# 1pathplanningzzj/pointnet_refine

Measured on AMD Instinct MI355X. Metric: lane segments/sec (fwd+bwd) at B=4096,N=1024; HBM GB/s vs roofline, higher is better.
Workload: dtype f32 (large GEMMs: 2xfp16-split MFMA, 3 products, fp32 accumulate); 1 GPU; LineRefineNet training step (fwd + deep-supervision L1 + bwd + Adam), B=4096/GPU, N=1024, M=32, C=4; global_batch=4096, points=1024, parallelism=dp1, decoder_chunk=4096

## Files before the change

### pointnet_refine_amd/csrc/prh_attn16.hpp

```cpp
#pragma once
#include "prh_attn.hpp"
#include "prh_gemm_h2.hpp"

namespace prh {

constexpr int A16_ROWB = 80;
constexpr int A16_IMG = 32 * A16_ROWB;

template <int PREC> struct A16 {
  static constexpr int NPL = PREC == 0 ? 2 : 1;
  using frag = typename std::conditional<PREC == 0, f16x8, bf16x8>::type;
};

template <int PREC>
__device__ __forceinline__ float a16_scale(const float (&x)[16]) {
  if constexpr (PREC != 0) return 1.f;
  float m = 0.f;
#pragma unroll
  for (int t = 0; t < 16; ++t) m = fmaxf(m, fabsf(x[t]));
#pragma unroll
  for (int o = 32; o > 0; o >>= 1) m = fmaxf(m, __shfl_xor(m, o));
  return pow2_scale(m);
}
__device__ __forceinline__ float a16_scale_acc(const f32x16& x) {
  float m = 0.f;
#pragma unroll
  for (int t = 0; t < 16; ++t) m = fmaxf(m, fabsf(x[t]));
#pragma unroll
  for (int o = 32; o > 0; o >>= 1) m = fmaxf(m, __shfl_xor(m, o));
  return pow2_scale(m);
}
template <int PREC, int NP>
__device__ __forceinline__ void a16_split(const float* x_, typename A16<PREC>::frag (&o)[NP], float S = 1.f) {
  if constexpr (PREC == 0 && NP == 1) {
    typedef float v2f __attribute__((ext_vector_type(2)));
    uint4 h;
    unsigned* hp = reinterpret_cast<unsigned*>(&h);
#pragma unroll
    for (int j = 0; j < 4; ++j) {
      v2f v = {x_[2 * j] * S, x_[2 * j + 1] * S};
      f16x2 hb = __builtin_convertvector(v, f16x2);
      hp[j] = __builtin_bit_cast(unsigned, hb);
    }
    o[0] = __builtin_bit_cast(f16x8, h);
  } else if constexpr (PREC == 0) {
    float x[8];
#pragma unroll
    for (int j = 0; j < 8; ++j) x[j] = x_[j] * S;
    uint4 h, l;
    split2h(x[0], x[1], h.x, l.x); split2h(x[2], x[3], h.y, l.y);
    split2h(x[4], x[5], h.z, l.z); split2h(x[6], x[7], h.w, l.w);
    o[0] = __builtin_bit_cast(f16x8, h);
    o[1] = __builtin_bit_cast(f16x8, l);
  } else {
    const uint4 h = make_uint4(pack_bf16x2(x_[0], x_[1]), pack_bf16x2(x_[2], x_[3]), pack_bf16x2(x_[4], x_[5]),
                               pack_bf16x2(x_[6], x_[7]));
    o[0] = __builtin_bit_cast(bf16x8, h);
  }
}
template <int PREC, int NA, int NB>
__device__ __forceinline__ f32x16 a16_mma(const typename A16<PREC>::frag (&a)[NA],
                                          const typename A16<PREC>::frag (&b)[NB], f32x16 c) {
  if constexpr (PREC == 0) {
    if constexpr (NA > 1) c = __builtin_amdgcn_mfma_f32_32x32x16_f16(a[NA - 1], b[0], c, 0, 0, 0);
    if constexpr (NB > 1) c = __builtin_amdgcn_mfma_f32_32x32x16_f16(a[0], b[NB - 1], c, 0, 0, 0);
    c = __builtin_amdgcn_mfma_f32_32x32x16_f16(a[0], b[0], c, 0, 0, 0);
  } else {
    c = __builtin_amdgcn_mfma_f32_32x32x16_bf16(a[0], b[0], c, 0, 0, 0);
  }
  return c;
}
__device__ __forceinline__ void a16_load_rows(const float* base, long ld, long row0, int rows_valid, int col0,
                                              int lane, float (&x)[16]) {
  const int r = lane & 31, h2 = lane >> 5;
  const bool ok = r < rows_valid;
  const float* p = base + (size_t)(row0 + (ok ? r : 0)) * ld + col0 + h2 * 8;
#pragma unroll
  for (int s = 0; s < 2; ++s)
#pragma unroll
    for (int j = 0; j < 2; ++j) {
      const float4 t = ok ? ldg4(p + s * 16 + 4 * j) : zero4();
      x[s * 8 + 4 * j] = t.x; x[s * 8 + 4 * j + 1] = t.y; x[s * 8 + 4 * j + 2] = t.z; x[s * 8 + 4 * j + 3] = t.w;
    }
}
template <bool KV16>
__device__ __forceinline__ void a16_load_kv(const float* base, long ld, long row0, int rows_valid, int col0,
                                            int lane, float (&x)[16]) {
  if constexpr (!KV16) {
    a16_load_rows(base, ld, row0, rows_valid, col0, lane, x);
  } else {
    const int r = lane & 31, h2 = lane >> 5;
    const bool ok = r < rows_valid;
    const unsigned short* p = reinterpret_cast<const unsigned short*>(base) + (size_t)(row0 + (ok ? r : 0)) * ld + col0 + h2 * 8;
#pragma unroll
    for (int s = 0; s < 2; ++s) {
      const uint4 u = ok ? *reinterpret_cast<const uint4*>(p + s * 16) : make_uint4(0u, 0u, 0u, 0u);
      x[s * 8 + 0] = bf16_lo(u.x); x[s * 8 + 1] = bf16_hi(u.x); x[s * 8 + 2] = bf16_lo(u.y); x[s * 8 + 3] = bf16_hi(u.y);
      x[s * 8 + 4] = bf16_lo(u.z); x[s * 8 + 5] = bf16_hi(u.z); x[s * 8 + 6] = bf16_lo(u.w); x[s * 8 + 7] = bf16_hi(u.w);
    }
  }
}
template <int PREC, int NP>
__device__ __forceinline__ void a16_store_rows(char* img, int lane, const typename A16<PREC>::frag (&f0)[NP],
                                               const typename A16<PREC>::frag (&f1)[NP]) {
  const int r = lane & 31, h2 = lane >> 5;
#pragma unroll
  for (int pl = 0; pl < NP; ++pl) {
    char* q = img + pl * A16_IMG + r * A16_ROWB + h2 * 16;
    *reinterpret_cast<uint4*>(q) = __builtin_bit_cast(uint4, f0[pl]);
    *reinterpret_cast<uint4*>(q + 32) = __builtin_bit_cast(uint4, f1[pl]);
  }
  asm volatile("" ::: "memory");
}
template <int PREC, int NP>
__device__ __forceinline__ void a16_tr(const char* img, int s, int lane, typename A16<PREC>::frag (&o)[NP]) {
  const int g = lane >> 4, j = lane & 15;
  const char* a = img + (16 * s + 4 * (g >> 1) + (j >> 2)) * A16_ROWB + (16 * (g & 1) + 4 * (j & 3)) * 2;
#pragma unroll
  for (int pl = 0; pl < NP; ++pl) {
    const fp16x4 lo = __builtin_amdgcn_ds_read_tr16_b64_v4f16((__attribute__((address_space(3))) fp16x4*)(a + pl * A16_IMG));
    const fp16x4 hi = __builtin_amdgcn_ds_read_tr16_b64_v4f16(
        (__attribute__((address_space(3))) fp16x4*)(a + pl * A16_IMG + 8 * A16_ROWB));
    struct Pair { fp16x4 a, b; } pr = {lo, hi};
    o[pl] = __builtin_bit_cast(typename A16<PREC>::frag, pr);
  }
}
template <int PREC, int NP>
__device__ __forceinline__ void a16_acc_frag(const f32x16& x, int s, typename A16<PREC>::frag (&o)[NP],
                                             float S = 1.f) {
  float t[8];
#pragma unroll
  for (int j = 0; j < 8; ++j) t[j] = x[8 * s + j];
  a16_split<PREC>(t, o, S);
}
__device__ __forceinline__ f32x16 a16_zero() {
  f32x16 z;
#pragma unroll
  for (int r = 0; r < 16; ++r) z[r] = 0.f;
  return z;
}

template <int PREC> constexpr int a16_fwd_wave_lds() {
  return A16<PREC>::NPL * A16_IMG > 18 * 64 * 4 ? A16<PREC>::NPL * A16_IMG : 18 * 64 * 4;
}
template <int PREC, bool KV16 = false>
__global__ __launch_bounds__(512) void attn16_fwd_kernel(const AttnParams p) {
  using frag = typename A16<PREC>::frag;
  constexpr int NPL = A16<PREC>::NPL;
  constexpr int NKV = KV16 ? 1 : NPL;
  constexpr int WL = a16_fwd_wave_lds<PREC>();
  extern __shared__ __attribute__((aligned(16))) char smem[];
  const int lane = threadIdx.x & 63, wave = threadIdx.x >> 6;
  const int h2 = lane >> 5, l31 = lane & 31;
  const int wpb = blockDim.x >> 6;
  const int hpb = p.H / wpb;
  const bool split = p.ksplit > 0;
  const int b = split ? blockIdx.x / p.H : blockIdx.x / hpb;
  const int h = split ? blockIdx.x % p.H : (blockIdx.x % hpb) * wpb + wave;
  const int kbeg = split ? wave * p.ksplit : 0;
  int kend = split ? kbeg + p.ksplit : p.N;
  kend = kend > p.N ? p.N : kend;
  const unsigned seed_eff = effective_seed(p.seed, p.seed_src);
  char* vimg = smem + wave * WL;
  const int col0 = h * 32;
  const unsigned bh = (unsigned)(b * p.H + h);

  for (int qt = 0; qt < p.M; qt += 32) {
    float x[16];
    a16_load_rows(p.q, p.ldq, (long)b * p.M + qt, p.M - qt, col0, lane, x);
#pragma unroll
    for (int t = 0; t < 16; ++t) x[t] *= p.scale;
    const float sq = a16_scale<PREC>(x);
    frag qf[2][NPL];
    a16_split<PREC>(x, qf[0], sq);
    a16_split<PREC>(x + 8, qf[1], sq);

    f32x16 oacc;
#pragma unroll
    for (int r = 0; r < 16; ++r) oacc[r] = 0.f;
    float m_run = -INFINITY, l_run = 0.f;

    float kn[16], vn[16];
    if (kbeg < kend) {
      a16_load_kv<KV16>(p.k, p.ldk, (long)b * p.N + kbeg, p.N - kbeg, col0, lane, kn);
      a16_load_kv<KV16>(p.v, p.ldv, (long)b * p.N + kbeg, p.N - kbeg, col0, lane, vn);
    }
    for (int k0 = kbeg; k0 < kend; k0 += 32) {
      frag kf[2][NKV], vf[2][NKV];
      const float sk = a16_scale<PREC>(kn), sv = a16_scale<PREC>(vn);
      a16_split<PREC>(kn, kf[0], sk); a16_split<PREC>(kn + 8, kf[1], sk);
      a16_split<PREC>(vn, vf[0], sv); a16_split<PREC>(vn + 8, vf[1], sv);
      if (k0 + 32 < kend) {
        a16_load_kv<KV16>(p.k, p.ldk, (long)b * p.N + k0 + 32, p.N - k0 - 32, col0, lane, kn);
        a16_load_kv<KV16>(p.v, p.ldv, (long)b * p.N + k0 + 32, p.N - k0 - 32, col0, lane, vn);
      }
      a16_store_rows<PREC>(vimg, lane, vf[0], vf[1]);
      f32x16 s = a16_zero();
      s = a16_mma<PREC>(kf[0], qf[0], s);
      s = a16_mma<PREC>(kf[1], qf[1], s);
      const float us = 1.f / (sk * sq);
      float mx = -INFINITY;
#pragma unroll
      for (int r = 0; r < 16; ++r) {
        s[r] = (k0 + crow(r, h2) >= p.N) ? -INFINITY : s[r] * us;
        mx = fmaxf(mx, s[r]);
      }
      mx = fmaxf(mx, __shfl_xor(mx, 32));
      const float m_new = fmaxf(m_run, mx);
      const float alpha = __expf(m_run - m_new);
      float psum = 0.f;
#pragma unroll
      for (int r = 0; r < 16; ++r) {
        const float e = __expf(s[r] - m_new);
        psum += e;
        float pd = e;
        if (p.drop_thresh != 0u)
          pd = attn_keep(seed_eff, bh, (unsigned)(qt + l31), (unsigned)(k0 + crow(r, h2)), p.drop_thresh)
                   ? e * p.keep_scale : 0.f;
        s[r] = pd;
        oacc[r] *= alpha;
      }
      psum += __shfl_xor(psum, 32);
      l_run = l_run * alpha + psum;
      m_run = m_new;
      f32x16 ot = a16_zero();
#pragma unroll
      for (int st = 0; st < 2; ++st) {
        frag pf[NPL], va[NKV];
        a16_acc_frag<PREC>(s, st, pf);
        a16_tr<PREC>(vimg, st, lane, va);
        ot = a16_mma<PREC>(va, pf, ot);
      }
      const float uv = 1.f / sv;
#pragma unroll
      for (int r = 0; r < 16; ++r) oacc[r] = fmaf(ot[r], uv, oacc[r]);
    }
    const int q = qt + l31;
    if (split) {
      asm volatile("" ::: "memory");
      float* part = reinterpret_cast<float*>(vimg);
#pragma unroll
      for (int r = 0; r < 16; ++r) part[r * 64 + lane] = oacc[r];
      part[16 * 64 + lane] = m_run;
      part[17 * 64 + lane] = l_run;
      __syncthreads();
      for (int g = wave; g < 4; g += wpb) {
        float mt = -INFINITY;
        for (int sw = 0; sw < wpb; ++sw) mt = fmaxf(mt, reinterpret_cast<const float*>(smem + sw * WL)[16 * 64 + lane]);
        float lt = 0.f;
        float4 ov = zero4();
        for (int sw = 0; sw < wpb; ++sw) {
          const float* ps = reinterpret_cast<const float*>(smem + sw * WL);
          const float ms = ps[16 * 64 + lane];
          const float w = ms == -INFINITY ? 0.f : __expf(ms - mt);
          lt = fmaf(ps[17 * 64 + lane], w, lt);
          ov.x = fmaf(ps[(4 * g) * 64 + lane], w, ov.x); ov.y = fmaf(ps[(4 * g + 1) * 64 + lane], w, ov.y);
          ov.z = fmaf(ps[(4 * g + 2) * 64 + lane], w, ov.z); ov.w = fmaf(ps[(4 * g + 3) * 64 + lane], w, ov.w);
        }
        const float inv = 1.f / lt;
        if (q < p.M) {
          float* op = p.o + (size_t)((long)b * p.M + q) * p.ldo + col0;
          *reinterpret_cast<float4*>(op + 8 * g + 4 * h2) = make_float4(ov.x * inv, ov.y * inv, ov.z * inv, ov.w * inv);
          if (g == 0 && h2 == 0) p.lse[((size_t)b * p.H + h) * p.M + q] = mt + __logf(lt);
        }
      }
      __syncthreads();
      continue;
    }
    const float inv = 1.f / l_run;
    if (q < p.M) {
      float* op = p.o + (size_t)((long)b * p.M + q) * p.ldo + col0;
#pragma unroll
      for (int g = 0; g < 4; ++g)
        *reinterpret_cast<float4*>(op + 8 * g + 4 * h2) =
            make_float4(oacc[4 * g] * inv, oacc[4 * g + 1] * inv, oacc[4 * g + 2] * inv, oacc[4 * g + 3] * inv);
      if (h2 == 0) p.lse[((size_t)b * p.H + h) * p.M + q] = m_run + __logf(l_run);
    }
  }
}

template <int PREC, bool KV16 = false, bool KSPLIT = false>
__global__ __launch_bounds__(KSPLIT ? 512 : 256, KSPLIT ? 1 : 2) void attn16_bwd_kernel(const AttnParams p) {
  using frag = typename A16<PREC>::frag;
  constexpr int NPL = A16<PREC>::NPL;
  constexpr int NKV = KV16 ? 1 : NPL;
  constexpr bool SCR_IN_DS = AT_TILE * 4 <= NPL * A16_IMG;
  constexpr int WAVE_LDS = 4 * NPL * A16_IMG + (SCR_IN_DS ? 0 : AT_TILE * 4);
  extern __shared__ __attribute__((aligned(16))) char dsm16[];
  const int lane = threadIdx.x & 63, wave = threadIdx.x >> 6;
  const int h2 = lane >> 5, l31 = lane & 31;
  const int wpb = blockDim.x >> 6;
  const int hpb = p.H / wpb;
  constexpr bool split = KSPLIT;
  const int b = split ? blockIdx.x / p.H : blockIdx.x / hpb;
  const int h = split ? blockIdx.x % p.H : (blockIdx.x % hpb) * wpb + wave;
  const int kbeg = split ? wave * p.ksplit : 0;
  int kend = split ? kbeg + p.ksplit : p.N;
  kend = kend > p.N ? p.N : kend;
  const unsigned seed_eff = effective_seed(p.seed, p.seed_src);
  char* qimg = dsm16 + wave * WAVE_LDS;
  char* doimg = qimg + NPL * A16_IMG;
  char* kimg = doimg + NPL * A16_IMG;
  char* dsimg = kimg + NPL * A16_IMG;
  float* scr = reinterpret_cast<float*>(SCR_IN_DS ? dsimg : dsimg + NPL * A16_IMG);
  const int col0 = h * 32;
  const unsigned bh = (unsigned)(b * p.H + h);
  float mx_dv = 0.f, mx_dk = 0.f;

  for (int qt = 0; qt < p.M; qt += 32) {
    float xq[16], xdo[16], xo[16];
    a16_load_rows(p.q, p.ldq, (long)b * p.M + qt, p.M - qt, col0, lane, xq);
    a16_load_rows(p.dout, p.lddo, (long)b * p.M + qt, p.M - qt, col0, lane, xdo);
    a16_load_rows(p.o, p.ldo, (long)b * p.M + qt, p.M - qt, col0, lane, xo);
#pragma unroll
    for (int t = 0; t < 16; ++t) xq[t] *= p.scale;
    const float sq = a16_scale<PREC>(xq), sdo = a16_scale<PREC>(xdo);
    frag qf[2][NPL], dof[2][NPL];
    a16_split<PREC>(xq, qf[0], sq); a16_split<PREC>(xq + 8, qf[1], sq);
    a16_split<PREC>(xdo, dof[0], sdo); a16_split<PREC>(xdo + 8, dof[1], sdo);
    a16_store_rows<PREC>(qimg, lane, qf[0], qf[1]);
    a16_store_rows<PREC>(doimg, lane, dof[0], dof[1]);
    float dl = 0.f;
#pragma unroll
    for (int t = 0; t < 16; ++t) dl = fmaf(xdo[t], xo[t], dl);
    dl += __shfl_xor(dl, 32);
    const int qcol = qt + l31;
    const float lse_col = qcol < p.M ? p.lse[((size_t)b * p.H + h) * p.M + qcol] : 0.f;
    const float dl_col = dl;
    if (h2 == 0) *reinterpret_cast<float2*>(qimg + l31 * A16_ROWB + 64) = make_float2(lse_col, dl_col);
    asm volatile("" ::: "memory");
    f32x16 dqacc;
#pragma unroll
    for (int r = 0; r < 16; ++r) dqacc[r] = 0.f;

    float kn[16], vn[16];
    if (kbeg < kend) {
      a16_load_kv<KV16>(p.k, p.ldk, (long)b * p.N + kbeg, p.N - kbeg, col0, lane, kn);
      a16_load_kv<KV16>(p.v, p.ldv, (long)b * p.N + kbeg, p.N - kbeg, col0, lane, vn);
    }
    for (int k0 = kbeg; k0 < kend; k0 += 32) {
      frag kf[2][NKV], vf[2][NKV];
      const float sk = a16_scale<PREC>(kn), sv = a16_scale<PREC>(vn);
      a16_split<PREC>(kn, kf[0], sk); a16_split<PREC>(kn + 8, kf[1], sk);
      a16_split<PREC>(vn, vf[0], sv); a16_split<PREC>(vn + 8, vf[1], sv);
      if (k0 + 32 < kend) {
        a16_load_kv<KV16>(p.k, p.ldk, (long)b * p.N + k0 + 32, p.N - k0 - 32, col0, lane, kn);
        a16_load_kv<KV16>(p.v, p.ldv, (long)b * p.N + k0 + 32, p.N - k0 - 32, col0, lane, vn);
      }
      a16_store_rows<PREC>(kimg, lane, kf[0], kf[1]);
      const bool key_ok = (k0 + l31) < p.N;
      const float us = 1.f / (sq * sk), udp = 1.f / (sdo * sv);

      f32x16 s = a16_zero(), dp = a16_zero();
#pragma unroll
      for (int st = 0; st < 2; ++st) {
        s = a16_mma<PREC>(qf[st], kf[st], s);
        dp = a16_mma<PREC>(dof[st], vf[st], dp);
      }
#pragma unroll
      for (int r = 0; r < 16; ++r) {
        const int q = qt + crow(r, h2);
        const float2 qs = *reinterpret_cast<const float2*>(qimg + crow(r, h2) * A16_ROWB + 64);
        float pr = (key_ok && q < p.M) ? __expf(s[r] * us - qs.x) : 0.f;
        float keepf = 1.f;
        if (p.drop_thresh != 0u)
          keepf = attn_keep(seed_eff, bh, (unsigned)q, (unsigned)(k0 + l31), p.drop_thresh) ? p.keep_scale : 0.f;
        const float ds = pr * (dp[r] * udp * keepf - qs.y);
        s[r] = pr * keepf;
        dp[r] = ds;
      }
      f32x16 dvt = a16_zero(), dkt = a16_zero();
      const float sds = PREC == 0 ? a16_scale_acc(dp) : 1.f;
#pragma unroll
      for (int st = 0; st < 2; ++st) {
        frag pf[NPL], dsf[NPL], at[NPL];
        a16_acc_frag<PREC>(s, st, pf);
        a16_tr<PREC>(doimg, st, lane, at);
        dvt = a16_mma<PREC>(at, pf, dvt);
        a16_acc_frag<PREC>(dp, st, dsf, sds);
        a16_tr<PREC>(qimg, st, lane, at);
        dkt = a16_mma<PREC>(at, dsf, dkt);
#pragma unroll
        for (int pl = 0; pl < NPL; ++pl) {
          const uint4 u = __builtin_bit_cast(uint4, dsf[pl]);
          char* q = dsimg + pl * A16_IMG + l31 * A16_ROWB + (16 * st + 4 * h2) * 2;
          *reinterpret_cast<uint2*>(q) = make_uint2(u.x, u.y);
          *reinterpret_cast<uint2*>(q + 16) = make_uint2(u.z, u.w);
        }
      }
      asm volatile("" ::: "memory");
      {
        const float uv = 1.f / sdo, uk = 1.f / (sq * sds);
#pragma unroll
        for (int r = 0; r < 16; ++r) { dvt[r] *= uv; dkt[r] *= uk; }
      }
      {
        f32x16 dqt = a16_zero();
#pragma unroll
        for (int st = 0; st < 2; ++st) {
          frag bt[NPL], at[NKV];
          a16_tr<PREC>(dsimg, st, lane, bt);
          a16_tr<PREC>(kimg, st, lane, at);
          dqt = a16_mma<PREC>(at, bt, dqt);
        }
        const float uq = 1.f / (sk * sds);
#pragma unroll
        for (int r = 0; r < 16; ++r) dqacc[r] = fmaf(dqt[r], uq, dqacc[r]);
      }
      asm volatile("" ::: "memory");
#pragma unroll
      for (int pass = 0; pass < 2; ++pass) {
        const f32x16& acc = pass == 0 ? dvt : dkt;
#pragma unroll
        for (int r = 0; r < 16; ++r) scr[l31 * AT_LD + crow(r, h2)] = acc[r];
        float* dst = pass == 0 ? p.dv : p.dk;
        const long ldd = pass == 0 ? p.lddv : p.lddk;
#pragma unroll
        for (int it = 0; it < 4; ++it) {
          const int key = (lane >> 3) + 8 * it;
          float4 vv = *reinterpret_cast<const float4*>(scr + key * AT_LD + (lane & 7) * 4);
          if (k0 + key < p.N) {
            const size_t eo = (size_t)((long)b * p.N + k0 + key) * ldd + col0 + (lane & 7) * 4;
            if constexpr (KV16) {
              uint2* gp = reinterpret_cast<uint2*>(reinterpret_cast<unsigned short*>(dst) + eo);
              if (qt > 0) {
                const uint2 old = *gp;
                vv.x += bf16_lo(old.x); vv.y += bf16_hi(old.x); vv.z += bf16_lo(old.y); vv.w += bf16_hi(old.y);
              }
              *gp = make_uint2(pack_bf16x2(vv.x, vv.y), pack_bf16x2(vv.z, vv.w));
            } else {
              float* gp = dst + eo;
              if (qt > 0) {
                const float4 old = ldg4(gp);
                vv.x += old.x; vv.y += old.y; vv.z += old.z; vv.w += old.w;
              }
              *reinterpret_cast<float4*>(gp) = vv;
            }
            const float m4 = fmaxf(fmaxf(fabsf(vv.x), fabsf(vv.y)), fmaxf(fabsf(vv.z), fabsf(vv.w)));
            if (pass == 0) mx_dv = fmaxf(mx_dv, m4); else mx_dk = fmaxf(mx_dk, m4);
          }
        }
      }
    }
    if (split) {
      asm volatile("" ::: "memory");
#pragma unroll
      for (int r = 0; r < 16; ++r) scr[r * 64 + lane] = dqacc[r];
      __syncthreads();
      for (int g = wave; g < 4 && qcol < p.M; g += wpb) {
        float4 dv4 = zero4();
        for (int sw = 0; sw < wpb; ++sw) {
          const float* ps = reinterpret_cast<const float*>(dsm16 + sw * WAVE_LDS + (scr - reinterpret_cast<float*>(qimg)) * 4);
          dv4.x += ps[(4 * g) * 64 + lane]; dv4.y += ps[(4 * g + 1) * 64 + lane];
          dv4.z += ps[(4 * g + 2) * 64 + lane]; dv4.w += ps[(4 * g + 3) * 64 + lane];
        }
        float* dqp = p.dq + (size_t)((long)b * p.M + qcol) * p.lddq + col0;
        *reinterpret_cast<float4*>(dqp + 8 * g + 4 * h2) =
            make_float4(dv4.x * p.scale, dv4.y * p.scale, dv4.z * p.scale, dv4.w * p.scale);
      }
      __syncthreads();
    } else if (qcol < p.M) {
      float* dqp = p.dq + (size_t)((long)b * p.M + qcol) * p.lddq + col0;
#pragma unroll
      for (int g = 0; g < 4; ++g)
        *reinterpret_cast<float4*>(dqp + 8 * g + 4 * h2) =
            make_float4(dqacc[4 * g] * p.scale, dqacc[4 * g + 1] * p.scale, dqacc[4 * g + 2] * p.scale,
                        dqacc[4 * g + 3] * p.scale);
    }
  }
  if (p.kv_amax_part != nullptr) {
#pragma unroll
    for (int o = 32; o > 0; o >>= 1) {
      mx_dv = fmaxf(mx_dv, __shfl_xor(mx_dv, o));
      mx_dk = fmaxf(mx_dk, __shfl_xor(mx_dk, o));
    }
    if (split) {
      float* red = reinterpret_cast<float*>(dsm16);
      if (lane == 0) { red[wave * 2] = mx_dv; red[wave * 2 + 1] = mx_dk; }
      __syncthreads();
      if (threadIdx.x == 0) {
        for (int sw = 1; sw < wpb; ++sw) { mx_dv = fmaxf(mx_dv, red[sw * 2]); mx_dk = fmaxf(mx_dk, red[sw * 2 + 1]); }
        p.kv_amax_part[(size_t)blockIdx.x * 2] = mx_dv;
        p.kv_amax_part[(size_t)blockIdx.x * 2 + 1] = mx_dk;
      }
    } else if (lane == 0) {
      p.kv_amax_part[(size_t)(blockIdx.x * wpb + wave) * 2] = mx_dv;
      p.kv_amax_part[(size_t)(blockIdx.x * wpb + wave) * 2 + 1] = mx_dk;
    }
  }
}

}
```

### pointnet_refine_amd/csrc/prh_lib.hip

```cpp
#include "../../include/pointnet_refine_hip.h"

#include <hip/hip_runtime.h>
#include <stdarg.h>
#include <stdio.h>
#include <string.h>

#include <mutex>
#include <vector>

#include <stdlib.h>

#include "prh_gemm.hpp"
#include "prh_attn.hpp"
#include "prh_attn16.hpp"
#include "prh_gemm_s3.hpp"
#include "prh_gemm_h2.hpp"
#include "prh_b16.hpp"
#include "prh_small.hpp"
#include "prh_attnfold.hpp"
#include "prh_fused.hpp"
#include "prh_context.hpp"
#include "prh_metrics.hpp"
#include "prh_drive.hpp"
#include "prh_match.hpp"
// ... 3459 lines not shown
                     double cell, const long long* cell_offsets, const int* rows, long long n_rows, double r2,
                     double reach, double z_lo, double bin, int n_bins, int min_points, int peak_num, int peak_den,
                     double* height, int* count, int* hits, int* bin_index, int device, void* stream) {
  TRY_RC(ground_check_grid("ground_query", points, is_double, slice_offsets, n_slices, n_points, grid_origin, grid_shape,
                           cell_base, n_cells, cell));
  if (n_queries < 0 || n_queries >= 4ll * 0x7fffffff || n_rows < 0 || n_rows > n_points)
    return fail(PRH_ERR_ARG, "ground_query: bad argument");
  if (!(r2 > 0.0) || !(r2 <= 16.0) || !(reach > 0.0) || !(reach * reach >= r2) || !(reach <= 8.0))
    return fail(PRH_ERR_ARG, "ground_query: 0 < radius <= 4 and radius <= reach <= 8");
  if (n_bins < 1 || n_bins > GROUND_MAX_BINS || !(bin > 0.0) || !(z_lo >= -256.0) || !(z_lo + n_bins * bin <= 256.0))
    return fail(PRH_ERR_ARG, "ground_query: 1 <= n_bins <= %d, bin > 0 and the histogram inside [-256, 256]",
                GROUND_MAX_BINS);
  if (min_points < 1 || peak_num < 1 || peak_num > peak_den || peak_den > 65536)
    return fail(PRH_ERR_ARG, "ground_query: min_points >= 1 and 1 <= peak_num <= peak_den <= 65536");
  if (n_queries == 0) return PRH_OK;
  if (!queries || !query_offsets || n_slices == 0 || !height || !count || !hits || !bin_index ||
      (n_cells > 0 && !cell_offsets) || (n_rows > 0 && !rows))
    return fail(PRH_ERR_ARG, "ground_query: null pointer");
  HIP_TRY(hipSetDevice(device));
  hipStream_t st = (hipStream_t)stream;
  GroundParams prm{r2, reach, cell, z_lo, bin, n_bins, min_points, peak_num, peak_den};
  const unsigned nblk = (unsigned)((n_queries + GROUND_WAVES - 1) / GROUND_WAVES);
  if (is_double)
    hipLaunchKernelGGL(ground_query_kernel<double>, dim3(nblk), dim3(GROUND_THREADS), 0, st, (const double*)points,
                       slice_offsets, n_slices, queries, query_offsets, n_queries, grid_origin, grid_shape, cell_base,
                       cell_offsets, rows, n_rows, n_cells, prm, height, count, hits, bin_index);
  else
    hipLaunchKernelGGL(ground_query_kernel<float>, dim3(nblk), dim3(GROUND_THREADS), 0, st, (const float*)points,
                       slice_offsets, n_slices, queries, query_offsets, n_queries, grid_origin, grid_shape, cell_base,
                       cell_offsets, rows, n_rows, n_cells, prm, height, count, hits, bin_index);
  LAUNCH_CHECK();
  return PRH_OK;
}

static bool attn_ksplit(int B, int H, int N, int& keys_per_wave) {
  keys_per_wave = 0;
  if ((long)B * H > 1024 || N < 128) return false;
  int nw = cdiv(N, 32) < 8 ? cdiv(N, 32) : 8;
  keys_per_wave = cdiv(cdiv(N, 32), nw) * 32;
  return true;
}
static int attn_prepare(AttnParams& a, float dropout_p) {
  a.seed_src = g_seed_src;
  if (dropout_p < 0.f || dropout_p >= 1.f) return fail(PRH_ERR_ARG, "attention: dropout_p must be in [0,1)");
  a.keep_scale = 1.f / (1.f - dropout_p);
  a.drop_thresh = dropout_p > 0.f ? (unsigned)((double)dropout_p * 4294967296.0) : 0u;
  if (!a.q || !a.k || !a.v || !a.o || !a.lse || a.B <= 0 || a.M <= 0 || a.N <= 0)
    return fail(PRH_ERR_ARG, "attention: bad argument");
  if (a.H <= 0 || a.H % 4) return fail(PRH_ERR_ARG, "attention: heads (%d) must be a multiple of 4", a.H);
  if ((a.ldq | a.ldk | a.ldv | a.ldo) & 3) return fail(PRH_ERR_ARG, "attention: leading dimensions must be multiples of 4");
  return PRH_OK;
}

static int attn_forward(AttnParams& a, bool kv16, int prec, float dropout_p, int device, hipStream_t st) {
  TRY(attn_prepare(a, dropout_p));
  HIP_TRY(hipSetDevice(device));
  const int B = a.B, M = a.M, N = a.N, H = a.H;
  ProfScope ps(prec < 0 ? "attn_fwd" : "attn16_fwd<split>",
               4.0 * B * H * (double)M * N * 32, 4.0 * (2.0 * B * N * H * 32 + 2.0 * B * M * H * 32), st);
  int wpb = (long)B * (H / 4) < 512 ? 1 : 4;
  if (kv16 && prec < 0) return fail(PRH_ERR_ARG, "attention: bf16 K/V need the 16-bit attention cores");
  unsigned grid = (unsigned)(B * (H / wpb));
  if (prec >= 0 && attn_ksplit(B, H, N, a.ksplit)) { wpb = cdiv(N, a.ksplit); grid = (unsigned)(B * H); }
  const size_t ldsf = (size_t)wpb * a16_fwd_wave_lds<0>();
  if (prec >= 0 && kv16)
    hipLaunchKernelGGL((attn16_fwd_kernel<0, true>), dim3(grid), dim3(64 * wpb), ldsf, st, a);
  else if (prec >= 0)
    hipLaunchKernelGGL(attn16_fwd_kernel<0>, dim3(grid), dim3(64 * wpb), ldsf, st, a);
  else
    hipLaunchKernelGGL(attn_fwd_kernel, dim3(grid), dim3(64 * wpb), 0, st, a);
  LAUNCH_CHECK();
  return PRH_OK;
}

static int attn_backward(AttnParams& a, bool kv16, int prec, float dropout_p, int device, hipStream_t st) {
  TRY(attn_prepare(a, dropout_p));
  if (!a.dout || !a.dq || !a.dk || !a.dv) return fail(PRH_ERR_ARG, "attention_backward: null gradient pointer");
  if ((a.lddo | a.lddq | a.lddk | a.lddv) & 3) return fail(PRH_ERR_ARG, "attention_backward: leading dimensions must be multiples of 4");
  HIP_TRY(hipSetDevice(device));
  const int B = a.B, M = a.M, N = a.N, H = a.H;
  int wpb = (long)B * (H / 4) < 512 ? 1 : 4;
  if (prec >= 0) {
    unsigned grid = (unsigned)(B * (H / wpb));
    if (attn_ksplit(B, H, N, a.ksplit)) { wpb = cdiv(N, a.ksplit); grid = (unsigned)(B * H); }
    const size_t lds16 = (size_t)wpb * 4 * 2 * A16_IMG;
    static const int attr16 = allow_big_lds(attn16_bwd_kernel<0>, attn16_bwd_kernel<0, true>);
    if (attr16 != PRH_OK) return attr16;
    const double kvb = kv16 ? 2.0 : 4.0;
    ProfScope ps("attn16_bwd<split>", 14.0 * B * H * (double)M * N * 32,
                 kvb * 4.0 * B * N * H * 32 + 4.0 * 4.0 * B * M * H * 32, st);
    if (a.ksplit > 0) {
      static const int attr16s = allow_big_lds(attn16_bwd_kernel<0, false, true>, attn16_bwd_kernel<0, true, true>);
      if (attr16s != PRH_OK) return attr16s;
      if (kv16)
        hipLaunchKernelGGL((attn16_bwd_kernel<0, true, true>), dim3(grid), dim3(64 * wpb), lds16, st, a);
      else
        hipLaunchKernelGGL((attn16_bwd_kernel<0, false, true>), dim3(grid), dim3(64 * wpb), lds16, st, a);
    } else if (kv16)
      hipLaunchKernelGGL((attn16_bwd_kernel<0, true>), dim3(grid), dim3(64 * wpb), lds16, st, a);
    else
      hipLaunchKernelGGL(attn16_bwd_kernel<0>, dim3(grid), dim3(64 * wpb), lds16, st, a);
    LAUNCH_CHECK();
    return PRH_OK;
  }
  const size_t lds = (size_t)wpb * 4 * AT_TILE * sizeof(float);
  static const int attr_rc = allow_big_lds(attn_bwd_kernel);
  if (attr_rc != PRH_OK) return attr_rc;
  ProfScope ps("attn_bwd", 14.0 * B * H * (double)M * N * 32, 4.0 * (4.0 * B * N * H * 32 + 4.0 * B * M * H * 32), st);
  hipLaunchKernelGGL(attn_bwd_kernel, dim3((unsigned)(B * (H / wpb))), dim3(64 * wpb), lds, st, a);
  LAUNCH_CHECK();
  return PRH_OK;
}

int prh_attn_forward(const float* q, long ldq, const float* k, long ldk, const float* v, long ldv,
                     float* o, long ldo, float* lse, int B, int M, int N, int H, float scale,
                     float dropout_p, unsigned seed, int device, void* stream) {
  AttnParams a; memset(&a, 0, sizeof(a));
  a.q = q; a.ldq = ldq; a.k = k; a.ldk = ldk; a.v = v; a.ldv = ldv; a.o = o; a.ldo = ldo; a.lse = lse;
  a.B = B; a.M = M; a.N = N; a.H = H; a.scale = scale; a.seed = seed;
  return attn_forward(a, false, cores_of(gemm_mode()).attn_prec(), dropout_p, device, (hipStream_t)stream);
}

int prh_attn_backward_ex(const float* q, long ldq, const float* k, long ldk, const float* v, long ldv,
                         const float* o, long ldo, const float* lse, const float* dout, long lddo,
                         float* dq, long lddq, float* dk, long lddk, float* dv, long lddv, int B, int M,
                         int N, int H, float scale, float dropout_p, unsigned seed, float* kv_amax_part,
                         int device, void* stream) {
  AttnParams a; memset(&a, 0, sizeof(a));
  a.kv_amax_part = kv_amax_part;
  a.q = q; a.ldq = ldq; a.k = k; a.ldk = ldk; a.v = v; a.ldv = ldv; a.o = (float*)o; a.ldo = ldo;
  a.lse = (float*)lse; a.dout = dout; a.lddo = lddo; a.dq = dq; a.lddq = lddq; a.dk = dk; a.lddk = lddk;
  a.dv = dv; a.lddv = lddv;
  a.B = B; a.M = M; a.N = N; a.H = H; a.scale = scale; a.seed = seed;
  return attn_backward(a, false, cores_of(gemm_mode()).attn_prec(), dropout_p, device, (hipStream_t)stream);
}
int prh_cast_perm_bf16(const float* src, long ld, uint16_t* dst, long rows, int device, void* stream) {
  if (!src || !dst || rows < 0 || ld < 256 || (ld & 3)) return fail(PRH_ERR_ARG, "cast_perm_bf16: bad argument");
  HIP_TRY(hipSetDevice(device));
  if (rows == 0) return PRH_OK;
  hipLaunchKernelGGL(cast_perm_b16_kernel, dim3((unsigned)cdiv(rows * 16, 256L)), dim3(256), 0, (hipStream_t)stream, src, ld,
                     dst, (size_t)rows);
  LAUNCH_CHECK();
  return PRH_OK;
}
int prh_posmem_images(const float* xyz, long ldx, const float* w0, const float* b0, const float* w2, const float* b2,
                      const float* memory, long ldm, long rows, uint16_t* x16, uint16_t* y16, int device, void* stream) {
  if (!xyz || !w0 || !w2 || !memory || !x16 || !y16 || rows < 0 || ldx < 3 || ldm < 256)
    return fail(PRH_ERR_ARG, "posmem_images: bad argument");
  HIP_TRY(hipSetDevice(device));
  if (rows == 0) return PRH_OK;
  static const int attr = allow_big_lds(posmem_images_kernel);
  if (attr != PRH_OK) return attr;
  static const int n_cu = [] {
    int dev = 0, cu = 256;
// ... 260 lines not shown
```

Before: 10020 segments/s.

## Use buffer loads, DPP/permlane reductions and compile-time dropout in 16-bit attention

Replaces shuffle-based wave max and half-wave reductions with DPP, readlane and permlane32_swap sequences. K/V/Q/gradient loads and stores move to raw buffer resources, whose hardware bounds checking replaces the per-row validity branches. Dropout becomes a template parameter so the no-dropout path compiles without RNG checks, and the backward precomputes keep bits. The grad store is factored into RMW and non-RMW variants. Adds an extent check limiting segments to 2 GiB and doubles the number of kernel instantiations.

After: 10110 segments/s, median of 6. Within noise of the previous version (+0.9%).

```diff
diff --git a/pointnet_refine_amd/csrc/prh_attn16.hpp b/pointnet_refine_amd/csrc/prh_attn16.hpp
--- a/pointnet_refine_amd/csrc/prh_attn16.hpp
+++ b/pointnet_refine_amd/csrc/prh_attn16.hpp
@@ -1,6 +1,7 @@
 #pragma once
 #include "prh_attn.hpp"
 #include "prh_gemm_h2.hpp"
+#include "prh_pow2.hpp"
 
 namespace prh {
 
@@ -12,23 +13,43 @@
   using frag = typename std::conditional<PREC == 0, f16x8, bf16x8>::type;
 };
 
+template <int CTRL>
+__device__ __forceinline__ float a16_dpp_max(float m) {
+  return fmaxf(m, __int_as_float(__builtin_amdgcn_update_dpp(0, __float_as_int(m), CTRL, 0xf, 0xf, false)));
+}
+__device__ __forceinline__ float a16_wave_max(float m) {
+  m = a16_dpp_max<0xB1>(m);
+  m = a16_dpp_max<0x4E>(m);
+  m = a16_dpp_max<0x141>(m);
+  m = a16_dpp_max<0x140>(m);
+  const int u = __float_as_int(m);
+  const unsigned r0 = (unsigned)__builtin_amdgcn_readlane(u, 0), r1 = (unsigned)__builtin_amdgcn_readlane(u, 16);
+  const unsigned r2 = (unsigned)__builtin_amdgcn_readlane(u, 32), r3 = (unsigned)__builtin_amdgcn_readlane(u, 48);
+  const unsigned a = r0 > r1 ? r0 : r1, b = r2 > r3 ? r2 : r3;
+  return __uint_as_float(a > b ? a : b);
+}
+__device__ __forceinline__ void a16_halves(float x, float& lo, float& hi) {
+  const auto r = __builtin_amdgcn_permlane32_swap(__float_as_uint(x), __float_as_uint(x), false, false);
+  lo = __uint_as_float(r[0]); hi = __uint_as_float(r[1]);
+}
+__device__ __forceinline__ float a16_half_sum(float x) { float lo, hi; a16_halves(x, lo, hi); return lo + hi; }
+__device__ __forceinline__ float a16_half_max(float x) { float lo, hi; a16_halves(x, lo, hi); return fmaxf(lo, hi); }
+__device__ __forceinline__ float a16_inv(float a) { return 1.f / a; }
+__device__ __forceinline__ float a16_inv(float a, float b) { return 1.f / (a * b); }
+
 template <int PREC>
 __device__ __forceinline__ float a16_scale(const float (&x)[16]) {
   if constexpr (PREC != 0) return 1.f;
   float m = 0.f;
 #pragma unroll
   for (int t = 0; t < 16; ++t) m = fmaxf(m, fabsf(x[t]));
-#pragma unroll
-  for (int o = 32; o > 0; o >>= 1) m = fmaxf(m, __shfl_xor(m, o));
-  return pow2_scale(m);
+  return __uint_as_float(pow2_scale_bits(__float_as_uint(a16_wave_max(m))));
 }
 __device__ __forceinline__ float a16_scale_acc(const f32x16& x) {
   float m = 0.f;
 #pragma unroll
   for (int t = 0; t < 16; ++t) m = fmaxf(m, fabsf(x[t]));
-#pragma unroll
-  for (int o = 32; o > 0; o >>= 1) m = fmaxf(m, __shfl_xor(m, o));
-  return pow2_scale(m);
+  return __uint_as_float(pow2_scale_bits(__float_as_uint(a16_wave_max(m))));
 }
 template <int PREC, int NP>
 __device__ __forceinline__ void a16_split(const float* x_, typename A16<PREC>::frag (&o)[NP], float S = 1.f) {
@@ -83,18 +104,29 @@
       x[s * 8 + 4 * j] = t.x; x[s * 8 + 4 * j + 1] = t.y; x[s * 8 + 4 * j + 2] = t.z; x[s * 8 + 4 * j + 3] = t.w;
     }
 }
-template <bool KV16>
-__device__ __forceinline__ void a16_load_kv(const float* base, long ld, long row0, int rows_valid, int col0,
-                                            int lane, float (&x)[16]) {
-  if constexpr (!KV16) {
-    a16_load_rows(base, ld, row0, rows_valid, col0, lane, x);
+__device__ __forceinline__ __amdgpu_buffer_rsrc_t a16_seg_rsrc(const void* base, long ld, int seg, int rows, int cols,
+                                                               int esz) {
+  const char* first = reinterpret_cast<const char*>(base) + (size_t)((long)seg * rows) * ld * esz;
+  return __builtin_amdgcn_make_buffer_rsrc(const_cast<char*>(first), 0, (int)((((long)rows - 1) * ld + cols) * esz),
+                                           0x00020000);
+}
+__device__ __forceinline__ int a16_lane_off(int ld, int row0, int col0, int lane, int esz) {
+  return ((row0 + (lane & 31)) * ld + col0 + (lane >> 5) * 8) * esz;
+}
+template <bool E16>
+__device__ __forceinline__ void a16_buf_rows(__amdgpu_buffer_rsrc_t rs, int vo, float (&x)[16]) {
+  if constexpr (!E16) {
+#pragma unroll
+    for (int s = 0; s < 2; ++s)
+#pragma unroll
+      for (int j = 0; j < 2; ++j) {
+        const float4 t = __builtin_bit_cast(float4, __builtin_amdgcn_raw_buffer_load_b128(rs, vo + s * 64 + j * 16, 0, 0));
+        x[s * 8 + 4 * j] = t.x; x[s * 8 + 4 * j + 1] = t.y; x[s * 8 + 4 * j + 2] = t.z; x[s * 8 + 4 * j + 3] = t.w;
+      }
   } else {
-    const int r = lane & 31, h2 = lane >> 5;
-    const bool ok = r < rows_valid;
-    const unsigned short* p = reinterpret_cast<const unsigned short*>(base) + (size_t)(row0 + (ok ? r : 0)) * ld + col0 + h2 * 8;
 #pragma unroll
     for (int s = 0; s < 2; ++s) {
-      const uint4 u = ok ? *reinterpret_cast<const uint4*>(p + s * 16) : make_uint4(0u, 0u, 0u, 0u);
+      const uint4 u = __builtin_bit_cast(uint4, __builtin_amdgcn_raw_buffer_load_b128(rs, vo + s * 32, 0, 0));
       x[s * 8 + 0] = bf16_lo(u.x); x[s * 8 + 1] = bf16_hi(u.x); x[s * 8 + 2] = bf16_lo(u.y); x[s * 8 + 3] = bf16_hi(u.y);
       x[s * 8 + 4] = bf16_lo(u.z); x[s * 8 + 5] = bf16_hi(u.z); x[s * 8 + 6] = bf16_lo(u.w); x[s * 8 + 7] = bf16_hi(u.w);
     }
@@ -143,7 +175,7 @@
 template <int PREC> constexpr int a16_fwd_wave_lds() {
   return A16<PREC>::NPL * A16_IMG > 18 * 64 * 4 ? A16<PREC>::NPL * A16_IMG : 18 * 64 * 4;
 }
-template <int PREC, bool KV16 = false>
+template <int PREC, bool KV16 = false, bool DROP = false>
 __global__ __launch_bounds__(512) void attn16_fwd_kernel(const AttnParams p) {
   using frag = typename A16<PREC>::frag;
   constexpr int NPL = A16<PREC>::NPL;
@@ -164,10 +196,16 @@
   char* vimg = smem + wave * WL;
   const int col0 = h * 32;
   const unsigned bh = (unsigned)(b * p.H + h);
+  constexpr int KVB = KV16 ? 2 : 4;
+  const __amdgpu_buffer_rsrc_t rq = a16_seg_rsrc(p.q, p.ldq, b, p.M, p.H * 32, 4);
+  const __amdgpu_buffer_rsrc_t rk = a16_seg_rsrc(p.k, p.ldk, b, p.N, p.H * 32, KVB);
+  const __amdgpu_buffer_rsrc_t rv = a16_seg_rsrc(p.v, p.ldv, b, p.N, p.H * 32, KVB);
+  const int ko = a16_lane_off((int)p.ldk, 0, col0, lane, KVB), vo = a16_lane_off((int)p.ldv, 0, col0, lane, KVB);
+  const int kstep = (int)p.ldk * KVB, vstep = (int)p.ldv * KVB;
 
   for (int qt = 0; qt < p.M; qt += 32) {
     float x[16];
-    a16_load_rows(p.q, p.ldq, (long)b * p.M + qt, p.M - qt, col0, lane, x);
+    a16_buf_rows<false>(rq, a16_lane_off((int)p.ldq, qt, col0, lane, 4), x);
 #pragma unroll
     for (int t = 0; t < 16; ++t) x[t] *= p.scale;
     const float sq = a16_scale<PREC>(x);
@@ -181,31 +219,33 @@
     float m_run = -INFINITY, l_run = 0.f;
 
     float kn[16], vn[16];
-    if (kbeg < kend) {
-      a16_load_kv<KV16>(p.k, p.ldk, (long)b * p.N + kbeg, p.N - kbeg, col0, lane, kn);
-      a16_load_kv<KV16>(p.v, p.ldv, (long)b * p.N + kbeg, p.N - kbeg, col0, lane, vn);
+    {
+      const int kr = kbeg < kend ? kbeg : p.N;
+      a16_buf_rows<KV16>(rk, ko + kr * kstep, kn);
+      a16_buf_rows<KV16>(rv, vo + kr * vstep, vn);
     }
     for (int k0 = kbeg; k0 < kend; k0 += 32) {
       frag kf[2][NKV], vf[2][NKV];
       const float sk = a16_scale<PREC>(kn), sv = a16_scale<PREC>(vn);
       a16_split<PREC>(kn, kf[0], sk); a16_split<PREC>(kn + 8, kf[1], sk);
       a16_split<PREC>(vn, vf[0], sv); a16_split<PREC>(vn + 8, vf[1], sv);
-      if (k0 + 32 < kend) {
-        a16_load_kv<KV16>(p.k, p.ldk, (long)b * p.N + k0 + 32, p.N - k0 - 32, col0, lane, kn);
-        a16_load_kv<KV16>(p.v, p.ldv, (long)b * p.N + k0 + 32, p.N - k0 - 32, col0, lane, vn);
+      {
+        const int kr = k0 + 32 < kend ? k0 + 32 : p.N;
+        a16_buf_rows<KV16>(rk, ko + kr * kstep, kn);
+        a16_buf_rows<KV16>(rv, vo + kr * vstep, vn);
       }
       a16_store_rows<PREC>(vimg, lane, vf[0], vf[1]);
       f32x16 s = a16_zero();
       s = a16_mma<PREC>(kf[0], qf[0], s);
       s = a16_mma<PREC>(kf[1], qf[1], s);
-      const float us = 1.f / (sk * sq);
+      const float us = a16_inv(sk, sq);
       float mx = -INFINITY;
 #pragma unroll
       for (int r = 0; r < 16; ++r) {
         s[r] = (k0 + crow(r, h2) >= p.N) ? -INFINITY : s[r] * us;
         mx = fmaxf(mx, s[r]);
       }
-      mx = fmaxf(mx, __shfl_xor(mx, 32));
+      mx = a16_half_max(mx);
       const float m_new = fmaxf(m_run, mx);
       const float alpha = __expf(m_run - m_new);
       float psum = 0.f;
@@ -214,13 +254,13 @@
         const float e = __expf(s[r] - m_new);
         psum += e;
         float pd = e;
-        if (p.drop_thresh != 0u)
+        if constexpr (DROP)
           pd = attn_keep(seed_eff, bh, (unsigned)(qt + l31), (unsigned)(k0 + crow(r, h2)), p.drop_thresh)
                    ? e * p.keep_scale : 0.f;
         s[r] = pd;
         oacc[r] *= alpha;
       }
-      psum += __shfl_xor(psum, 32);
+      psum = a16_half_sum(psum);
       l_run = l_run * alpha + psum;
       m_run = m_new;
       f32x16 ot = a16_zero();
@@ -231,7 +271,7 @@
         a16_tr<PREC>(vimg, st, lane, va);
         ot = a16_mma<PREC>(va, pf, ot);
       }
-      const float uv = 1.f / sv;
+      const float uv = a16_inv(sv);
 #pragma unroll
       for (int r = 0; r < 16; ++r) oacc[r] = fmaf(ot[r], uv, oacc[r]);
     }
@@ -279,7 +319,38 @@
   }
 }
 
-template <int PREC, bool KV16 = false, bool KSPLIT = false>
+template <bool G16, bool RMW>
+__device__ __forceinline__ float a16_store_grad(const f32x16& acc, float* scr, __amdgpu_buffer_rsrc_t rs, int vo,
+                                                int step8, int lane, int keys_valid, float mx) {
+  const int l31 = lane & 31, h2 = lane >> 5;
+#pragma unroll
+  for (int r = 0; r < 16; ++r) scr[l31 * AT_LD + crow(r, h2)] = acc[r];
+#pragma unroll
+  for (int it = 0; it < 4; ++it) {
+    const int key = (lane >> 3) + 8 * it;
+    float4 vv = *reinterpret_cast<const float4*>(scr + key * AT_LD + (lane & 7) * 4);
+    const int off = vo + it * step8;
+    if constexpr (G16) {
+      if constexpr (RMW) {
+        const uint2 old = __builtin_bit_cast(uint2, __builtin_amdgcn_raw_buffer_load_b64(rs, off, 0, 0));
+        vv.x += bf16_lo(old.x); vv.y += bf16_hi(old.x); vv.z += bf16_lo(old.y); vv.w += bf16_hi(old.y);
+      }
+      __builtin_amdgcn_raw_buffer_store_b64(
+          __builtin_bit_cast(v2i_t, make_uint2(pack_bf16x2(vv.x, vv.y), pack_bf16x2(vv.z, vv.w))), rs, off, 0, 0);
+    } else {
+      if constexpr (RMW) {
+        const float4 old = __builtin_bit_cast(float4, __builtin_amdgcn_raw_buffer_load_b128(rs, off, 0, 0));
+        vv.x += old.x; vv.y += old.y; vv.z += old.z; vv.w += old.w;
+      }
+      __builtin_amdgcn_raw_buffer_store_b128(__builtin_bit_cast(u32x4, vv), rs, off, 0, 0);
+    }
+    const float m4 = fmaxf(fmaxf(fabsf(vv.x), fabsf(vv.y)), fmaxf(fabsf(vv.z), fabsf(vv.w)));
+    mx = fmaxf(mx, key < keys_valid ? m4 : 0.f);
+  }
+  return mx;
+}
+
+template <int PREC, bool KV16 = false, bool KSPLIT = false, bool DROP = false>
 __global__ __launch_bounds__(KSPLIT ? 512 : 256, KSPLIT ? 1 : 2) void attn16_bwd_kernel(const AttnParams p) {
   using frag = typename A16<PREC>::frag;
   constexpr int NPL = A16<PREC>::NPL;
@@ -306,12 +377,28 @@
   const int col0 = h * 32;
   const unsigned bh = (unsigned)(b * p.H + h);
   float mx_dv = 0.f, mx_dk = 0.f;
+  constexpr int KVB = KV16 ? 2 : 4;
+  const int cols = p.H * 32;
+  const __amdgpu_buffer_rsrc_t rk = a16_seg_rsrc(p.k, p.ldk, b, p.N, cols, KVB);
+  const __amdgpu_buffer_rsrc_t rv = a16_seg_rsrc(p.v, p.ldv, b, p.N, cols, KVB);
+  const __amdgpu_buffer_rsrc_t rdk = a16_seg_rsrc(p.dk, p.lddk, b, p.N, cols, KVB);
+  const __amdgpu_buffer_rsrc_t rdv = a16_seg_rsrc(p.dv, p.lddv, b, p.N, cols, KVB);
+  const int ko = a16_lane_off((int)p.ldk, 0, col0, lane, KVB), vo = a16_lane_off((int)p.ldv, 0, col0, lane, KVB);
+  const int kstep = (int)p.ldk * KVB, vstep = (int)p.ldv * KVB;
+  const int dkstep = (int)p.lddk * KVB, dvstep = (int)p.lddv * KVB;
+  const int dko = ((lane >> 3) * (int)p.lddk + col0 + (lane & 7) * 4) * KVB;
+  const int dvo = ((lane >> 3) * (int)p.lddv + col0 + (lane & 7) * 4) * KVB;
 
   for (int qt = 0; qt < p.M; qt += 32) {
     float xq[16], xdo[16], xo[16];
-    a16_load_rows(p.q, p.ldq, (long)b * p.M + qt, p.M - qt, col0, lane, xq);
-    a16_load_rows(p.dout, p.lddo, (long)b * p.M + qt, p.M - qt, col0, lane, xdo);
-    a16_load_rows(p.o, p.ldo, (long)b * p.M + qt, p.M - qt, col0, lane, xo);
+    {
+      const __amdgpu_buffer_rsrc_t rq = a16_seg_rsrc(p.q, p.ldq, b, p.M, cols, 4);
+      const __amdgpu_buffer_rsrc_t rdo = a16_seg_rsrc(p.dout, p.lddo, b, p.M, cols, 4);
+      const __amdgpu_buffer_rsrc_t ro = a16_seg_rsrc(p.o, p.ldo, b, p.M, cols, 4);
+      a16_buf_rows<false>(rq, a16_lane_off((int)p.ldq, qt, col0, lane, 4), xq);
+      a16_buf_rows<false>(rdo, a16_lane_off((int)p.lddo, qt, col0, lane, 4), xdo);
+      a16_buf_rows<false>(ro, a16_lane_off((int)p.ldo, qt, col0, lane, 4), xo);
+    }
 #pragma unroll
     for (int t = 0; t < 16; ++t) xq[t] *= p.scale;
     const float sq = a16_scale<PREC>(xq), sdo = a16_scale<PREC>(xdo);
@@ -323,9 +410,9 @@
     float dl = 0.f;
 #pragma unroll
     for (int t = 0; t < 16; ++t) dl = fmaf(xdo[t], xo[t], dl);
-    dl += __shfl_xor(dl, 32);
+    dl = a16_half_sum(dl);
     const int qcol = qt + l31;
-    const float lse_col = qcol < p.M ? p.lse[((size_t)b * p.H + h) * p.M + qcol] : 0.f;
+    const float lse_col = qcol < p.M ? p.lse[((size_t)b * p.H + h) * p.M + qcol] : INFINITY;
     const float dl_col = dl;
     if (h2 == 0) *reinterpret_cast<float2*>(qimg + l31 * A16_ROWB + 64) = make_float2(lse_col, dl_col);
     asm volatile("" ::: "memory");
@@ -334,22 +421,24 @@
     for (int r = 0; r < 16; ++r) dqacc[r] = 0.f;
 
     float kn[16], vn[16];
-    if (kbeg < kend) {
-      a16_load_kv<KV16>(p.k, p.ldk, (long)b * p.N + kbeg, p.N - kbeg, col0, lane, kn);
-      a16_load_kv<KV16>(p.v, p.ldv, (long)b * p.N + kbeg, p.N - kbeg, col0, lane, vn);
+    {
+      const int kr = kbeg < kend ? kbeg : p.N;
+      a16_buf_rows<KV16>(rk, ko + kr * kstep, kn);
+      a16_buf_rows<KV16>(rv, vo + kr * vstep, vn);
     }
     for (int k0 = kbeg; k0 < kend; k0 += 32) {
       frag kf[2][NKV], vf[2][NKV];
       const float sk = a16_scale<PREC>(kn), sv = a16_scale<PREC>(vn);
       a16_split<PREC>(kn, kf[0], sk); a16_split<PREC>(kn + 8, kf[1], sk);
       a16_split<PREC>(vn, vf[0], sv); a16_split<PREC>(vn + 8, vf[1], sv);
-      if (k0 + 32 < kend) {
-        a16_load_kv<KV16>(p.k, p.ldk, (long)b * p.N + k0 + 32, p.N - k0 - 32, col0, lane, kn);
-        a16_load_kv<KV16>(p.v, p.ldv, (long)b * p.N + k0 + 32, p.N - k0 - 32, col0, lane, vn);
+      {
+        const int kr = k0 + 32 < kend ? k0 + 32 : p.N;
+        a16_buf_rows<KV16>(rk, ko + kr * kstep, kn);
+        a16_buf_rows<KV16>(rv, vo + kr * vstep, vn);
       }
       a16_store_rows<PREC>(kimg, lane, kf[0], kf[1]);
       const bool key_ok = (k0 + l31) < p.N;
-      const float us = 1.f / (sq * sk), udp = 1.f / (sdo * sv);
+      const float us = a16_inv(sq, sk), udp = a16_inv(sdo, sv);
 
       f32x16 s = a16_zero(), dp = a16_zero();
 #pragma unroll
@@ -357,16 +446,24 @@
         s = a16_mma<PREC>(qf[st], kf[st], s);
         dp = a16_mma<PREC>(dof[st], vf[st], dp);
       }
+      unsigned keep_bits = 0u;
+      if constexpr (DROP) {
+        unsigned qb = (unsigned)(qt + 4 * h2);
+        asm volatile("" : "+v"(qb));
+#pragma unroll
+        for (int r = 0; r < 16; ++r)
+          keep_bits |= (attn_keep(seed_eff, bh, qb + (unsigned)crow(r, 0), (unsigned)(k0 + l31), p.drop_thresh) ? 1u : 0u) << r;
+      }
 #pragma unroll
       for (int r = 0; r < 16; ++r) {
-        const int q = qt + crow(r, h2);
         const float2 qs = *reinterpret_cast<const float2*>(qimg + crow(r, h2) * A16_ROWB + 64);
-        float pr = (key_ok && q < p.M) ? __expf(s[r] * us - qs.x) : 0.f;
+        float pr = key_ok ? __expf(s[r] * us - qs.x) : 0.f;
         float keepf = 1.f;
-        if (p.drop_thresh != 0u)
-          keepf = attn_keep(seed_eff, bh, (unsigned)q, (unsigned)(k0 + l31), p.drop_thresh) ? p.keep_scale : 0.f;
+        if constexpr (DROP) keepf = (keep_bits >> r) & 1u ? p.keep_scale : 0.f;
         const float ds = pr * (dp[r] * udp * keepf - qs.y);
-        s[r] = pr * keepf;
+        float pd = pr * keepf;
+        if constexpr (DROP) asm("" : "+v"(pd));
+        s[r] = pd;
         dp[r] = ds;
       }
       f32x16 dvt = a16_zero(), dkt = a16_zero();
@@ -390,7 +487,7 @@
       }
       asm volatile("" ::: "memory");
       {
-        const float uv = 1.f / sdo, uk = 1.f / (sq * sds);
+        const float uv = a16_inv(sdo), uk = a16_inv(sq, sds);
 #pragma unroll
         for (int r = 0; r < 16; ++r) { dvt[r] *= uv; dkt[r] *= uk; }
       }
@@ -403,43 +500,17 @@
           a16_tr<PREC>(kimg, st, lane, at);
           dqt = a16_mma<PREC>(at, bt, dqt);
         }
-        const float uq = 1.f / (sk * sds);
+        const float uq = a16_inv(sk, sds);
 #pragma unroll
         for (int r = 0; r < 16; ++r) dqacc[r] = fmaf(dqt[r], uq, dqacc[r]);
       }
       asm volatile("" ::: "memory");
-#pragma unroll
-      for (int pass = 0; pass < 2; ++pass) {
-        const f32x16& acc = pass == 0 ? dvt : dkt;
-#pragma unroll
-        for (int r = 0; r < 16; ++r) scr[l31 * AT_LD + crow(r, h2)] = acc[r];
-        float* dst = pass == 0 ? p.dv : p.dk;
-        const long ldd = pass == 0 ? p.lddv : p.lddk;
-#pragma unroll
-        for (int it = 0; it < 4; ++it) {
-          const int key = (lane >> 3) + 8 * it;
-          float4 vv = *reinterpret_cast<const float4*>(scr + key * AT_LD + (lane & 7) * 4);
-          if (k0 + key < p.N) {
-            const size_t eo = (size_t)((long)b * p.N + k0 + key) * ldd + col0 + (lane & 7) * 4;
-            if constexpr (KV16) {
-              uint2* gp = reinterpret_cast<uint2*>(reinterpret_cast<unsigned short*>(dst) + eo);
-              if (qt > 0) {
-                const uint2 old = *gp;
-                vv.x += bf16_lo(old.x); vv.y += bf16_hi(old.x); vv.z += bf16_lo(old.y); vv.w += bf16_hi(old.y);
-              }
-              *gp = make_uint2(pack_bf16x2(vv.x, vv.y), pack_bf16x2(vv.z, vv.w));
-            } else {
-              float* gp = dst + eo;
-              if (qt > 0) {
-                const float4 old = ldg4(gp);
-                vv.x += old.x; vv.y += old.y; vv.z += old.z; vv.w += old.w;
-              }
-              *reinterpret_cast<float4*>(gp) = vv;
-            }
-            const float m4 = fmaxf(fmaxf(fabsf(vv.x), fabsf(vv.y)), fmaxf(fabsf(vv.z), fabsf(vv.w)));
-            if (pass == 0) mx_dv = fmaxf(mx_dv, m4); else mx_dk = fmaxf(mx_dk, m4);
-          }
-        }
+      if (qt > 0) {
+        mx_dv = a16_store_grad<KV16, true>(dvt, scr, rdv, dvo + k0 * dvstep, 8 * dvstep, lane, p.N - k0, mx_dv);
+        mx_dk = a16_store_grad<KV16, true>(dkt, scr, rdk, dko + k0 * dkstep, 8 * dkstep, lane, p.N - k0, mx_dk);
+      } else {
+        mx_dv = a16_store_grad<KV16, false>(dvt, scr, rdv, dvo + k0 * dvstep, 8 * dvstep, lane, p.N - k0, mx_dv);
+        mx_dk = a16_store_grad<KV16, false>(dkt, scr, rdk, dko + k0 * dkstep, 8 * dkstep, lane, p.N - k0, mx_dk);
       }
     }
     if (split) {
@@ -469,11 +540,8 @@
     }
   }
   if (p.kv_amax_part != nullptr) {
-#pragma unroll
-    for (int o = 32; o > 0; o >>= 1) {
-      mx_dv = fmaxf(mx_dv, __shfl_xor(mx_dv, o));
-      mx_dk = fmaxf(mx_dk, __shfl_xor(mx_dk, o));
-    }
+    mx_dv = a16_wave_max(mx_dv);
+    mx_dk = a16_wave_max(mx_dk);
     if (split) {
       float* red = reinterpret_cast<float*>(dsm16);
       if (lane == 0) { red[wave * 2] = mx_dv; red[wave * 2 + 1] = mx_dk; }
diff --git a/pointnet_refine_amd/csrc/prh_lib.hip b/pointnet_refine_amd/csrc/prh_lib.hip
--- a/pointnet_refine_amd/csrc/prh_lib.hip
+++ b/pointnet_refine_amd/csrc/prh_lib.hip
@@ -3535,6 +3535,16 @@
   return PRH_OK;
 }
 
+static int attn16_check_extents(const AttnParams& a, bool kv16, bool backward) {
+  const long cols = (long)a.H * 32, kvb = kv16 ? 2 : 4, lim = 0x7fffffffl;
+  auto fits = [&](long ld, long rows, long esz) { return ld >= cols && ((rows + 32) * ld + cols) * esz <= lim; };
+  bool ok = fits(a.ldq, a.M, 4) && fits(a.ldk, a.N, kvb) && fits(a.ldv, a.N, kvb);
+  if (backward)
+    ok = ok && fits(a.lddo, a.M, 4) && fits(a.ldo, a.M, 4) && fits(a.lddk, a.N, kvb) && fits(a.lddv, a.N, kvb);
+  if (!ok) return fail(PRH_ERR_ARG, "attention: a leading dimension below H*32, or a segment of 2 GiB or more");
+  return PRH_OK;
+}
+
 static int attn_forward(AttnParams& a, bool kv16, int prec, float dropout_p, int device, hipStream_t st) {
   TRY(attn_prepare(a, dropout_p));
   HIP_TRY(hipSetDevice(device));
@@ -3546,10 +3556,16 @@
   unsigned grid = (unsigned)(B * (H / wpb));
   if (prec >= 0 && attn_ksplit(B, H, N, a.ksplit)) { wpb = cdiv(N, a.ksplit); grid = (unsigned)(B * H); }
   const size_t ldsf = (size_t)wpb * a16_fwd_wave_lds<0>();
-  if (prec >= 0 && kv16)
-    hipLaunchKernelGGL((attn16_fwd_kernel<0, true>), dim3(grid), dim3(64 * wpb), ldsf, st, a);
+  if (prec >= 0) TRY(attn16_check_extents(a, kv16, false));
+  const bool drop = a.drop_thresh != 0u;
+  if (prec >= 0 && kv16 && drop)
+    hipLaunchKernelGGL((attn16_fwd_kernel<0, true, true>), dim3(grid), dim3(64 * wpb), ldsf, st, a);
+  else if (prec >= 0 && kv16)
+    hipLaunchKernelGGL((attn16_fwd_kernel<0, true, false>), dim3(grid), dim3(64 * wpb), ldsf, st, a);
+  else if (prec >= 0 && drop)
+    hipLaunchKernelGGL((attn16_fwd_kernel<0, false, true>), dim3(grid), dim3(64 * wpb), ldsf, st, a);
   else if (prec >= 0)
-    hipLaunchKernelGGL(attn16_fwd_kernel<0>, dim3(grid), dim3(64 * wpb), ldsf, st, a);
+    hipLaunchKernelGGL((attn16_fwd_kernel<0, false, false>), dim3(grid), dim3(64 * wpb), ldsf, st, a);
   else
     hipLaunchKernelGGL(attn_fwd_kernel, dim3(grid), dim3(64 * wpb), 0, st, a);
   LAUNCH_CHECK();
@@ -3567,22 +3583,28 @@
     unsigned grid = (unsigned)(B * (H / wpb));
     if (attn_ksplit(B, H, N, a.ksplit)) { wpb = cdiv(N, a.ksplit); grid = (unsigned)(B * H); }
     const size_t lds16 = (size_t)wpb * 4 * 2 * A16_IMG;
-    static const int attr16 = allow_big_lds(attn16_bwd_kernel<0>, attn16_bwd_kernel<0, true>);
+    TRY(attn16_check_extents(a, kv16, true));
+    static const int attr16 = allow_big_lds(
+        attn16_bwd_kernel<0, false, false, false>, attn16_bwd_kernel<0, false, false, true>,
+        attn16_bwd_kernel<0, true, false, false>, attn16_bwd_kernel<0, true, false, true>,
+        attn16_bwd_kernel<0, false, true, false>, attn16_bwd_kernel<0, false, true, true>,
+        attn16_bwd_kernel<0, true, true, false>, attn16_bwd_kernel<0, true, true, true>);
     if (attr16 != PRH_OK) return attr16;
     const double kvb = kv16 ? 2.0 : 4.0;
     ProfScope ps("attn16_bwd<split>", 14.0 * B * H * (double)M * N * 32,
                  kvb * 4.0 * B * N * H * 32 + 4.0 * 4.0 * B * M * H * 32, st);
-    if (a.ksplit > 0) {
-      static const int attr16s = allow_big_lds(attn16_bwd_kernel<0, false, true>, attn16_bwd_kernel<0, true, true>);
-      if (attr16s != PRH_OK) return attr16s;
-      if (kv16)
-        hipLaunchKernelGGL((attn16_bwd_kernel<0, true, true>), dim3(grid), dim3(64 * wpb), lds16, st, a);
-      else
-        hipLaunchKernelGGL((attn16_bwd_kernel<0, false, true>), dim3(grid), dim3(64 * wpb), lds16, st, a);
-    } else if (kv16)
-      hipLaunchKernelGGL((attn16_bwd_kernel<0, true>), dim3(grid), dim3(64 * wpb), lds16, st, a);
-    else
-      hipLaunchKernelGGL(attn16_bwd_kernel<0>, dim3(grid), dim3(64 * wpb), lds16, st, a);
+    const int variant = (kv16 ? 4 : 0) | (a.ksplit > 0 ? 2 : 0) | (a.drop_thresh != 0u ? 1 : 0);
+    const dim3 g(grid), blk(64 * wpb);
+    switch (variant) {
+      case 0: hipLaunchKernelGGL((attn16_bwd_kernel<0, false, false, false>), g, blk, lds16, st, a); break;
+      case 1: hipLaunchKernelGGL((attn16_bwd_kernel<0, false, false, true>), g, blk, lds16, st, a); break;
+      case 2: hipLaunchKernelGGL((attn16_bwd_kernel<0, false, true, false>), g, blk, lds16, st, a); break;
+      case 3: hipLaunchKernelGGL((attn16_bwd_kernel<0, false, true, true>), g, blk, lds16, st, a); break;
+      case 4: hipLaunchKernelGGL((attn16_bwd_kernel<0, true, false, false>), g, blk, lds16, st, a); break;
+      case 5: hipLaunchKernelGGL((attn16_bwd_kernel<0, true, false, true>), g, blk, lds16, st, a); break;
+      case 6: hipLaunchKernelGGL((attn16_bwd_kernel<0, true, true, false>), g, blk, lds16, st, a); break;
+      default: hipLaunchKernelGGL((attn16_bwd_kernel<0, true, true, true>), g, blk, lds16, st, a); break;
+    }
     LAUNCH_CHECK();
     return PRH_OK;
   }
diff --git a/pointnet_refine_amd/csrc/prh_pow2.hpp b/pointnet_refine_amd/csrc/prh_pow2.hpp
--- /dev/null
+++ b/pointnet_refine_amd/csrc/prh_pow2.hpp
@@ -0,0 +1,20 @@
+#pragma once
+#include <stdint.h>
+
+#if defined(__HIPCC__) || defined(__CUDACC__)
+#define PRH_HD __host__ __device__ __forceinline__
+#else
+#define PRH_HD inline
+#endif
+
+namespace prh {
+
+PRH_HD uint32_t pow2_scale_bits(uint32_t amax) {
+  const int e = (int)((amax >> 23) & 0xffu);
+  int se = 267 - e;
+  se = se < 67 ? 67 : (se > 187 ? 187 : se);
+  const uint32_t plain = 0u - (uint32_t)((unsigned)(e - 1) < 254u);
+  return (((uint32_t)se << 23) & plain) | (0x3F800000u & ~plain);
+}
+
+}
```
